# HarryShomer/LPFormer

Measured on AMD Instinct MI355X. Metric: candidate link-pairs scored/sec (whole node), higher is better.
Workload: dtype f32

## Files before the change

include/lpformer_hip.h:

```cpp
#ifndef LPFORMER_HIP_H
#define LPFORMER_HIP_H

#include <stdint.h>

#ifdef __cplusplus
extern "C" {
#endif

#define LPF_OK 0
#define LPF_ERR_INVALID (-1)
#define LPF_ERR_UNSUPPORTED (-2)
#define LPF_ERR_LAUNCH (-3)
#define LPF_ERR_NO_DEVICE (-4)

#define LPF_ABI_VERSION 16

#define LPF_FLAG_RELU 1u

int lpf_abi_version(void);
const char *lpf_strerror(int code);
const char *lpf_last_hip_error(void);
int lpf_device_info(int *cu_count, int *lds_bytes_per_cu, int *wave_size, char *arch_name, int arch_name_len);


// ... 89 lines not shown
                     const void *adj_cv, const void *a1_cv, const void *px_cv, const void *t0_cv, int32_t mode_cn,
                     int32_t use_px, void *desc, int64_t *offs, int32_t *item_pair, int64_t item_cap, int64_t *ctl,
                     uint64_t *plan_lb, void *stream);
int lpf_select3_run(int64_t bs, const void *desc, const int64_t *offs, const int32_t *item_pair, int64_t item_cap,
                    int64_t *ctl, uint64_t *run_lb, const void *u_cv, const void *mini, float th_cn, float th_1hop,
                    float th_non1hop, int32_t mode_cn, int32_t *type_ptr, void *entries, int64_t ent_cap,
                    int32_t grid_blocks, void *stream);

#define LPF_SELECT4_BLOCK 64
#define LPF_SELECT4_CTL_WORDS 32
int lpf_select4(int64_t bs, const int64_t *batch, int64_t batch_ld, int64_t n_nodes, const void *node_rec,
                const void *adj_cv, const void *a1_cv, const void *px_cv, const void *t0_cv, const void *u_cv,
                const void *mini, int32_t mode_cn, int32_t use_px, float th_cn, float th_1hop, float th_non1hop,
                int64_t *ctl, void *pair_tab, int32_t *blk_cnt, void *blk_types, void *entries, int64_t ent_cap,
                int32_t threads, void *stream);

int lpf_select4_regions(int64_t bs, const void *pair_tab, const void *blk_types, const void *entries4, int64_t ent_cap4,
                        int32_t *type_ptr, void *regions, int64_t ent_cap, int64_t *ctl, void *stream);

int lpf_select_export(int64_t bs, const int32_t *type_ptr, const void *entries, int64_t ent_cap, int64_t *type_ptr64,
                      float *counts_f, int64_t ldc, int32_t n_counts, int32_t *sel_pair, int32_t *sel_node,
                      float *sel_pa, float *sel_pb, void *stream);

int lpf_pair_scores_f32(int32_t D, const int64_t *type_ptr, int64_t bs, const int32_t *sel_pair,
                        const int32_t *sel_node, const float *sel_pa, const float *sel_pb,
                        const float *Z, int64_t ldz, const float *q, int64_t ldq,
                        const float *pe_tab, const float *pe_stat, const float *wfold_packed, const float *bfold,
                        const float *att, float *score, int64_t max_entries, void *stream);

int lpf_pair_softmax_gather_f32(int32_t D, int64_t bs, const int64_t *type_ptr, const int32_t *sel_node,
// ... 120 lines not shown
                                   float *pieces, int64_t units_cap, float *out, int64_t ldo, int32_t *perm,
                                   int64_t *n_nonempty, void *stream);

int lpf_tail_chain_rows_perm_f32(int64_t M, int32_t D, int32_t n_counts, const float *rows, int64_t ldrows,
                                 const float *wB_packed, const float *bB, const float *lnB_g, const float *lnB_b,
                                 const float *r_e, int64_t ldre, const float *wC_packed, const float *bC,
                                 const float *w_dot, const float *b_dot, const int64_t *sel_ctl, const int32_t *perm,
                                 const int64_t *n_full, const float *bC_empty, const float *row_empty, float *logit,
                                 float *prob, void *stream);
int lpf_tail_chain_rows_perm_bf16(int64_t M, int32_t D, int32_t n_counts, const float *rows, int64_t ldrows,
                                  const void *wB_packed_bf16, const float *bB, const float *lnB_g, const float *lnB_b,
                                  const float *r_e, int64_t ldre, const void *wC_packed_bf16, const float *bC,
                                  const float *w_dot, const float *b_dot, const int64_t *sel_ctl, const int32_t *perm,
                                  const int64_t *n_full, const float *bC_empty, const float *row_empty, float *logit,
                                  float *prob, void *stream);

int lpf_rowdot_sigmoid_f32(int64_t M, int32_t K, const float *A, int64_t lda, const float *w, float b,
                           float *logit, float *prob, void *stream);


int64_t lpf_ppr_push_workspace_bytes(int64_t n, int64_t n_waves, double alpha, double eps);

int lpf_ppr_push_f64(int64_t n, const int64_t *rowptr, const int32_t *col, double alpha, double eps,
                     int64_t n_waves, void *workspace, int64_t workspace_bytes, int32_t *pool_col, float *pool_val,
                     int64_t pool_capacity, int64_t *row_off, int32_t *row_len, int64_t *counters, void *stream);

int lpf_ppr_push_f64_sources(int64_t n, const int64_t *rowptr, const int32_t *col, int64_t n_src,
                             const int32_t *sources, double alpha, double eps, int64_t n_waves, void *workspace,
                             int64_t workspace_bytes, int32_t *pool_col, float *pool_val, int64_t pool_capacity,
                             int64_t *row_off, int32_t *row_len, int64_t *counters, void *stream);
// ... 149 lines not shown
```

lpformer_amd/csrc/select4.hip:

```cpp
#include "walk_common.h"

namespace {

using namespace walk;

constexpr int S4_PAIRS = LPF_SELECT4_BLOCK;
#ifndef S4_ROUNDS_N
#define S4_ROUNDS_N 4
#endif
constexpr int S4_ROUNDS = S4_ROUNDS_N;
constexpr int CTL_SLOTS = 1, CTL_ERR = 3, CTL_DONE = 10, CTL_ALLOC = 16;
constexpr int S4_SHARDS = 8;
static_assert(CTL_ALLOC + S4_SHARDS <= LPF_SELECT4_CTL_WORDS, "control block too small");

struct Args4 {
    int64_t bs;
    const int64_t *batch;
    int64_t batch_ld, n_nodes;
    const NodeRec *rec;
    const int2 *adj_cv, *a1_cv, *px_cv, *t0_cv;
    const int2 *u_cv;
    const uint32_t *mini;
    int32_t mode_cn, use_px;
    float th_cn, th_1, th_n;
    int64_t *ctl;
    int4 *pair_tab;
    int32_t *blk_cnt;
    int4 *blk_types;
    int4 *entries;
    int64_t ent_cap;
};

template <int NTH, int NB>
struct Lds4 {
    static constexpr int WAVES = NTH / 64, NR = WAVES * S4_ROUNDS, PAIRS = S4_PAIRS * NB;
    PairDesc3 dsc[PAIRS];
    uint4 flt[PAIRS][2][MINI_WORDS / 4];
    int32_t sflag[WAVES][S4_ROUNDS][64];
    int32_t loc[PAIRS];
    int32_t pcnt[PAIRS][4];
    int32_t rcnt[NR];
    int32_t sub[NB];
    int64_t base;
    int32_t run, ovf;
};
// ... 196 lines not shown
        for (int r = 0; r < S4_ROUNDS; ++r) {
            const int g = WAVES * r + wave;
            const int c3 = code[r] & 3;
            const int pos = L.rcnt[g < NR ? g : 0] + __popcll(keptb[r] & lt_mask);
            if (c3 && !ovf)
                A.entries[base + pos] = make_int4((int32_t)((uint32_t)(p0 + win[r]) | ((uint32_t)c3 << 29) |
                                                            ((code[r] & 4) ? FROM_B : 0u)),
                                                  node[r], __float_as_int(va[r]), __float_as_int(vb[r]));
            if (first[r]) L.pcnt[win[r]][3] = pos;
        }
    }
    S4_STAMP(8);
    lpf_lds_barrier();
    S4_STAMP(9);
    const bool ovf = S > 0 && L.ovf != 0;
    if (wave < NB) {
        const int j = S4_PAIRS * wave + lane;
        const int4 cc = *reinterpret_cast<const int4 *>(L.pcnt[j]);
        int kept = (j < np && !ovf) ? cc.x + cc.y + cc.z : 0;
        const int ne = __popcll(__ballot(kept > 0));
#pragma unroll
        for (int dlt = 32; dlt > 0; dlt >>= 1) kept += __shfl_xor(kept, dlt, 64);
        const int64_t blk = (int64_t)blockIdx.x * NB + wave;
        if (lane == 0 && blk * S4_PAIRS < A.bs) reinterpret_cast<int2 *>(A.blk_cnt)[blk] = make_int2(kept, ne);
        if (A.blk_types) {
            int c0 = (j < np && !ovf) ? cc.x : 0, c1 = (j < np && !ovf) ? cc.y : 0, c2 = (j < np && !ovf) ? cc.z : 0;
#pragma unroll
            for (int dlt = 32; dlt > 0; dlt >>= 1) {
                c0 += __shfl_xor(c0, dlt, 64);
                c1 += __shfl_xor(c1, dlt, 64);
                c2 += __shfl_xor(c2, dlt, 64);
            }
            if (lane == 0 && blk * S4_PAIRS < A.bs) A.blk_types[blk] = make_int4(c0, c1, c2, 0);
        }
    }
    if (tid < np) {
        const int4 c = *reinterpret_cast<const int4 *>(L.pcnt[tid]);
        A.pair_tab[p0 + tid] = ovf ? make_int4(0, 0, 0, 0) : make_int4((int32_t)(L.base + c.w), c.x, c.y, c.z);
    }
    if (tid == 0) {
        if (ovf) atomicOr(reinterpret_cast<unsigned long long *>(A.ctl + CTL_ERR), (unsigned long long)LPF_SELECT_ERR_ENTRY_CAP);
        const unsigned long long done = atomicAdd(reinterpret_cast<unsigned long long *>(A.ctl + CTL_DONE), 1ull);
        if (done == (unsigned long long)gridDim.x - 1ull) {
            unsigned long long most = 0ull, sum = 0ull;
            for (int sh = 0; sh < S4_SHARDS; ++sh) {
                const unsigned long long v = atomicExch(reinterpret_cast<unsigned long long *>(A.ctl + CTL_ALLOC + sh), 0ull);
                most = v > most ? v : most;
                sum += v;
            }
            atomicExch(reinterpret_cast<unsigned long long *>(A.ctl + CTL_DONE), 0ull);
            A.ctl[0] = (int64_t)(most * S4_SHARDS);
            A.ctl[CTL_SLOTS] = (int64_t)sum;
        }
// ... 4 lines not shown
        uint64_t *o = s4_stamp_buf + (int64_t)blockIdx.x * 16;
        for (int k = 0; k < 11; ++k) o[k] = st_t[k];
        o[11] = (uint64_t)S;
    }
#endif
}

}

#ifdef S4_STAMPS
extern "C" int lpf_select4_set_stamps(void *buf) {
    return hipMemcpyToSymbol(HIP_SYMBOL(s4_stamp_buf), &buf, sizeof(buf)) == hipSuccess ? LPF_OK : LPF_ERR_LAUNCH;
}
#endif

extern "C" int lpf_select4(int64_t bs, const int64_t *batch, int64_t batch_ld, int64_t n_nodes, const void *node_rec,
                           const void *adj_cv, const void *a1_cv, const void *px_cv, const void *t0_cv, const void *u_cv,
                           const void *mini, int32_t mode_cn, int32_t use_px, float th_cn, float th_1hop,
                           float th_non1hop, int64_t *ctl, void *pair_tab, int32_t *blk_cnt, void *blk_types,
                           void *entries, int64_t ent_cap, int32_t threads, void *stream) {
    if (bs == 0) return LPF_OK;
    LPF_REQUIRE(bs > 0 && bs < (1ll << 29) && batch && batch_ld >= bs && n_nodes > 0 && node_rec && adj_cv && a1_cv &&
                (px_cv || !use_px) && u_cv && mini && ctl && pair_tab && blk_cnt && entries && ent_cap > 0 &&
                ent_cap < (1ll << 31) && lpf_aligned16(node_rec) && lpf_aligned16(u_cv) && lpf_aligned16(mini) &&
                lpf_aligned16(pair_tab) && lpf_aligned16(entries) && (reinterpret_cast<uintptr_t>(blk_cnt) & 7) == 0 &&
                lpf_aligned16(blk_types));
    Args4 a;
    a.bs = bs; a.batch = batch; a.batch_ld = batch_ld; a.n_nodes = n_nodes;
    a.rec = static_cast<const NodeRec *>(node_rec);
    a.adj_cv = static_cast<const int2 *>(adj_cv); a.a1_cv = static_cast<const int2 *>(a1_cv);
    a.px_cv = static_cast<const int2 *>(px_cv); a.t0_cv = static_cast<const int2 *>(t0_cv);
    a.u_cv = static_cast<const int2 *>(u_cv); a.mini = static_cast<const uint32_t *>(mini);
    a.mode_cn = mode_cn; a.use_px = use_px; a.th_cn = th_cn; a.th_1 = th_1hop; a.th_n = th_non1hop;
    a.ctl = ctl; a.pair_tab = static_cast<int4 *>(pair_tab); a.blk_cnt = blk_cnt;
    a.blk_types = static_cast<int4 *>(blk_types);
    a.entries = static_cast<int4 *>(entries); a.ent_cap = ent_cap;
    const int64_t nb = (bs + S4_PAIRS - 1) / S4_PAIRS;
    hipStream_t s = static_cast<hipStream_t>(stream);
    if (threads == 0) {
        const int n_cu = lpf_cu_count();
        if (n_cu == 0) return LPF_ERR_NO_DEVICE;
        threads = 1024 + ((nb + 1) / 2 >= n_cu ? 4096 : 0);
    }
    const int nth = threads & 4095, per = threads / 4096 + 1;
    const dim3 grid((unsigned)((nb + per - 1) / per));
    if (nth == 1024 && per == 2) hipLaunchKernelGGL((select4_kernel<1024, 2>), grid, dim3(1024), 0, s, a);
    else if (nth == 1024 && per == 1) hipLaunchKernelGGL((select4_kernel<1024, 1>), grid, dim3(1024), 0, s, a);
    else if (nth == 1024 && per == 4) hipLaunchKernelGGL((select4_kernel<1024, 4>), grid, dim3(1024), 0, s, a);
    else if (nth == 512 && per == 1) hipLaunchKernelGGL((select4_kernel<512, 1>), grid, dim3(512), 0, s, a);
    else if (nth == 512 && per == 2) hipLaunchKernelGGL((select4_kernel<512, 2>), grid, dim3(512), 0, s, a);
    else if (nth == 256 && per == 1) hipLaunchKernelGGL((select4_kernel<256, 1>), grid, dim3(256), 0, s, a);
    else return LPF_ERR_INVALID;
    LPF_CHECK_LAUNCH();
    return LPF_OK;
}

namespace {

struct ArgsR {
    int64_t bs;
    const int4 *pair_tab, *blk_types, *entries4;
    int64_t ent_cap4;
    int32_t *type_ptr;
    int4 *regions;
    int64_t ent_cap;
    int64_t *ctl;
};

__global__ __launch_bounds__(64) void s4_regions_kernel(const ArgsR A) {
// ... 98 lines not shown
```

lpformer_amd/csrc/tail_chain.hip:

```cpp
#include <type_traits>

#include "lpf_common.h"

namespace {

typedef float f32x4 __attribute__((ext_vector_type(4)));

#ifndef LPF_TC_GROUPS
#define LPF_TC_GROUPS 4
#endif
constexpr int TC_GROUPS = LPF_TC_GROUPS;
constexpr int TC_WAVES = 2 * TC_GROUPS;
constexpr int TC_THREADS = 64 * TC_WAVES;

struct TailArgs {
    int64_t M;
    const float *x; int64_t ldx; int KA;
    const float *addend; int64_t ldadd;
    const float *wA, *lnA_g, *lnA_b; int NA;
    const float *tail; int64_t ldtail;
    const float *wB, *bB, *lnB_g, *lnB_b; int NB;
    const float *re; int64_t ldre;
    const float *wC, *bC; int NC;
    const float *wdot, *bdot;
    float *logit, *prob;
    const float *part;
    const float *bnd;
    int64_t units_cap;
    const int32_t *type_ptr;
    const float *att_bias;
    const int64_t *sel_ctl;
    int n_counts;
    const float *rows; int64_t ldrows;
    const int32_t *perm;
    const int64_t *n_full;
    const float *bC_empty;
    const float *row_empty;
};

constexpr int tc_per_thread(int ntp) { return (ntp * 64 + TC_THREADS - 1) / TC_THREADS; }
constexpr int tc_stage_stride(int ntp) { return (ntp * 64 + 511) / 512 * 512; }

typedef short bf16x4_bits __attribute__((ext_vector_type(4)));
template <int P, int NTP, typename T>
__device__ __forceinline__ void tc_load(T (&r)[P], const float *packed, int stage, int tid) {
    const T *src = reinterpret_cast<const T *>(packed) + (int64_t)stage * tc_stage_stride(NTP);
#pragma unroll
    for (int e = 0; e < P; ++e) {
        const int i = e * TC_THREADS + tid;
#ifdef TC_NOWLOAD
        r[e] = T{};
        (void)src; (void)i;
// ... 61 lines not shown
#pragma unroll
    for (int c = 0; c < TPW; ++c) {
        const f32x4 gg = *reinterpret_cast<const f32x4 *>(g + fbase + 16 * c);
        const f32x4 bb = *reinterpret_cast<const f32x4 *>(b + fbase + 16 * c);
        acc[c] = (acc[c] - mean) * rstd * gg + bb;
        if (relu) {
#pragma unroll
            for (int r = 0; r < 4; ++r) acc[c][r] = fmaxf(acc[c][r], 0.f);
        }
    }
}

#ifdef TC_STAMPS
__device__ uint64_t *tc_stamp_buf = nullptr;
#define TC_STAMP(k) do { if (lane == 0) st_t[k] = wall_clock64(); } while (0)
#define TC_STAMPS_OUT(kind) do { if (lane == 0 && tc_stamp_buf) { uint64_t *o__ = tc_stamp_buf + ((int64_t)blockIdx.x * TC_WAVES + wave) * 8; \
        for (int k__ = 0; k__ < 7; ++k__) o__[k__] = st_t[k__]; o__[7] = (kind); } } while (0)
#else
#define TC_STAMP(k) do { } while (0)
#define TC_STAMPS_OUT(kind) do { } while (0)
#endif

template <int NTA, int NTB, int NTC>
struct TcShape {
    static constexpr int NTPA = (NTA + 1) & ~1, NTPB = (NTB + 1) & ~1, NTPC = (NTC + 1) & ~1;
    static constexpr int PA = tc_per_thread(NTPA), PB = tc_per_thread(NTPB), PC = tc_per_thread(NTPC);
    static constexpr int PM = PA > PB ? (PA > PC ? PA : PC) : (PB > PC ? PB : PC);
    static constexpr int SLAB = PM * TC_THREADS;
    static constexpr int HT = NTPA > NTPB ? NTPA : NTPB;
    static constexpr int HID = TC_GROUPS * HT * 64;
    static constexpr size_t BYTES = (size_t)(2 * SLAB + HID) * sizeof(f32x4) + TC_WAVES * 16 * sizeof(float);
};

template <int NTA, int NTB, int NTC, int WM = 0, bool ROWS = false>
__global__ __launch_bounds__(TC_THREADS, NTC >= 32 ? 2 : (TC_THREADS >= 512 ? 4 : 3)) void tail_chain_kernel(const TailArgs A) {
    using S = TcShape<NTA, NTB, NTC>;
    constexpr bool WB = WM != 0;
    using WT = typename std::conditional<WM == 1, uint2, f32x4>::type;
    constexpr int NTPA = S::NTPA, NTPB = S::NTPB, NTPC = S::NTPC;
    constexpr int TPWA = NTPA / 2, TPWB = NTPB / 2, TPWC = NTPC / 2;
    constexpr int NGE = NTA;
    extern __shared__ __attribute__((aligned(16))) f32x4 lds[];
    f32x4 *hid = lds + 2 * S::SLAB;
    float *xch = reinterpret_cast<float *>(hid + S::HID);
    const int tid = threadIdx.x, lane = tid & 63, wave = tid >> 6;
    const int grp = wave >> 1, half = wave & 1, q = lane >> 4, j = lane & 15;
    float *my_x = xch + wave * 16 + j;
    const float *peer_x = xch + (wave ^ 1) * 16 + j;
    f32x4 *my_hid = hid + (grp * S::HT) * 64 + lane;
// ... 6 lines not shown
    const int64_t tile = blockIdx.x;
    const int64_t pos = tile * (16 * TC_GROUPS) + grp * 16 + j;
    const bool live = pos < A.M;
    bool lite = false;
    int64_t m = pos;
    if constexpr (ROWS) {
        if (A.perm) {
            m = A.perm[live ? pos : A.M - 1];
            lite = tile * (16 * TC_GROUPS) >= *A.n_full;
        }
    }
    const int64_t mm = live ? m : (ROWS && A.perm ? m : A.M - 1);
    bool no_sel = false;
    if constexpr (ROWS) no_sel = A.perm && A.row_empty && (live ? pos : A.M - 1) >= *A.n_full;

    if constexpr (ROWS) {
        if (lite) {
            f32x4 acc[TPWC];
#pragma unroll
            for (int c = 0; c < TPWC; ++c) acc[c] = (f32x4){0.f, 0.f, 0.f, 0.f};
            WT wr[S::PC];
            const float *rer = A.re + mm * A.ldre + 4 * q;
            tc_load<S::PC, NTPC>(wr, A.wC, 0, tid);
            f32x4 xr = *reinterpret_cast<const f32x4 *>(rer);
#pragma unroll 1
            for (int kg = 0; kg < NGE; ++kg) {
                const f32x4 bv = xr;
                WT *lw = reinterpret_cast<WT *>(lds) + buf * S::SLAB;
                tc_store<S::PC>(wr, lw, tid);
                __syncthreads();
                if (kg + 1 < NGE) {
                    tc_load<S::PC, NTPC>(wr, A.wC, kg + 1, tid);
                    xr = *reinterpret_cast<const f32x4 *>(rer + 16 * (kg + 1));
                }
                tc_mfma<TPWC>(acc, lw + (half * TPWC) * 64 + lane, bv);
                buf ^= 1;
            }
            const int fbase = 16 * half * TPWC + 4 * q;
            float d = 0.f;
#pragma unroll
            for (int c = 0; c < TPWC; ++c) {
                const f32x4 b = *reinterpret_cast<const f32x4 *>(A.bC_empty + fbase + 16 * c);
                const f32x4 w = *reinterpret_cast<const f32x4 *>(A.wdot + fbase + 16 * c);
#pragma unroll
                for (int r = 0; r < 4; ++r) d = fmaf(fmaxf(acc[c][r] + b[r], 0.f), w[r], d);
            }
            d = lpf_quad_sum(d);
            if (q == 0) *my_x = d;
            __syncthreads();
            if (live && q == 0 && half == 0) {
                d = d + *peer_x + A.bdot[0];
// ... 152 lines not shown
            }
        }
#pragma unroll
        for (int kg = 0; kg < NTPA + 1; ++kg) {
            WT *lw = reinterpret_cast<WT *>(lds) + buf * S::SLAB;
            tc_store<S::PB>(wrB, lw, tid);
            __syncthreads();
            if (kg + 1 < NTPA + 1) tc_load<S::PB, NTPB>(wrB, A.wB, kg + 1, tid);
            const f32x4 bv = kg < NTPA ? my_hid[(kg < NTPA ? kg : 0) * 64] : tailv;
            tc_mfma<TPWB>(accB, lw + (half * TPWB) * 64 + lane, bv, !((NTB & 1) && half == 1));
            buf ^= 1;
        }
    }
    TC_STAMP(2);
    WT wrC[S::PC];
    tc_load<S::PC, NTPC>(wrC, A.wC, 0, tid);
    const float *rer = A.re + mm * A.ldre + 4 * q;
    f32x4 xr = *reinterpret_cast<const f32x4 *>(rer);
    {
        const int fbase = 16 * half * TPWB + 4 * q;
#pragma unroll
        for (int c = 0; c < TPWB; ++c) accB[c] += *reinterpret_cast<const f32x4 *>(A.bB + fbase + 16 * c);
        tc_layernorm<TPWB>(accB, fbase, A.NB, A.lnB_g, A.lnB_b, half, q, my_x, peer_x, true);
#pragma unroll
        for (int c = 0; c < TPWB; ++c) my_hid[(half * TPWB + c) * 64] = accB[c];
    }

    TC_STAMP(3);
    f32x4 accC[TPWC];
#pragma unroll
    for (int c = 0; c < TPWC; ++c) accC[c] = (f32x4){0.f, 0.f, 0.f, 0.f};
#pragma unroll 1
    for (int kg = 0; kg < NGE; ++kg) {
        const f32x4 bv = xr;
        WT *lw = reinterpret_cast<WT *>(lds) + buf * S::SLAB;
        tc_store<S::PC>(wrC, lw, tid);
        __syncthreads();
        tc_load<S::PC, NTPC>(wrC, A.wC, kg + 1, tid);
        if (kg + 1 < NGE) xr = *reinterpret_cast<const f32x4 *>(rer + 16 * (kg + 1));
        tc_mfma<TPWC>(accC, lw + (half * TPWC) * 64 + lane, bv);
        buf ^= 1;
    }
    TC_STAMP(4);
#pragma unroll
    for (int kg = 0; kg < NTB; ++kg) {
        WT *lw = reinterpret_cast<WT *>(lds) + buf * S::SLAB;
        tc_store<S::PC>(wrC, lw, tid);
        __syncthreads();
        if (kg + 1 < NTB) tc_load<S::PC, NTPC>(wrC, A.wC, NGE + kg + 1, tid);
        tc_mfma<TPWC>(accC, lw + (half * TPWC) * 64 + lane, my_hid[kg * 64]);
        buf ^= 1;
    }
    TC_STAMP(5);
    {
        const int fbase = 16 * half * TPWC + 4 * q;
        float d = 0.f;
#pragma unroll
        for (int c = 0; c < TPWC; ++c) {
// ... 5 lines not shown
        d = lpf_quad_sum(d);
        __syncthreads();
        if (q == 0) *my_x = d;
        __syncthreads();
        if (live && q == 0 && half == 0) {
            d = d + *peer_x + A.bdot[0];
            if (A.sel_ctl && A.sel_ctl[3] != 0) d = __builtin_nanf("");
            if (A.logit) A.logit[m] = d;
            if (A.prob) A.prob[m] = 1.0f / (1.0f + expf(-d));
        }
    }
    TC_STAMP(6);
    TC_STAMPS_OUT(0);
}

template <int NTA, int NTB, int NTC, int WM = 0, bool ROWS = false>
int tc_launch(const TailArgs &a, hipStream_t s) {
    constexpr size_t lds = TcShape<NTA, NTB, NTC>::BYTES;
    auto kern = tail_chain_kernel<NTA, NTB, NTC, WM, ROWS>;
    LPF_SET_MAX_LDS(kern, lds);
    const int64_t blocks = (a.M + 16 * TC_GROUPS - 1) / (16 * TC_GROUPS);
    if (blocks > 0x7fffffff) return LPF_ERR_UNSUPPORTED;
    hipLaunchKernelGGL(kern, dim3((unsigned)blocks), dim3(TC_THREADS), lds, s, a);
    LPF_CHECK_LAUNCH();
    return LPF_OK;
}

}

#ifdef TC_STAMPS
extern "C" int lpf_tail_chain_set_stamps(void *buf) {
    return hipMemcpyToSymbol(HIP_SYMBOL(tc_stamp_buf), &buf, sizeof(buf)) == hipSuccess ? LPF_OK : LPF_ERR_LAUNCH;
}
#endif
// ... 137 lines not shown
    return tc_rows<0>(M, D, n_counts, rows, ldrows, wB_packed, bB, lnB_g, lnB_b, r_e, ldre, wC_packed, bC, w_dot, b_dot,
                          sel_ctl, logit, prob, stream, perm, n_full, bC_empty, row_empty);
}

extern "C" int lpf_tail_chain_rows_perm_bf16(int64_t M, int32_t D, int32_t n_counts, const float *rows, int64_t ldrows,
                                             const void *wB_packed_bf16, const float *bB, const float *lnB_g,
                                             const float *lnB_b, const float *r_e, int64_t ldre,
                                             const void *wC_packed_bf16, const float *bC, const float *w_dot,
                                             const float *b_dot, const int64_t *sel_ctl, const int32_t *perm,
                                             const int64_t *n_full, const float *bC_empty, const float *row_empty,
                                             float *logit, float *prob, void *stream) {
    LPF_REQUIRE(perm && n_full && bC_empty);
    return tc_rows<1>(M, D, n_counts, rows, ldrows, wB_packed_bf16, bB, lnB_g, lnB_b, r_e, ldre, wC_packed_bf16, bC, w_dot,
                         b_dot, sel_ctl, logit, prob, stream, perm, n_full, bC_empty, row_empty);
}
```

lpformer_amd/link_transformer.py:

```python
from __future__ import annotations

import functools
import math
import weakref
from typing import Optional

import numpy as np
import torch
import torch.nn as nn

from . import _lib, fold, graph, mask_delta, ops, patterns
from . import dist as lpf_dist
from ._lib import FLAG_RELU, check, ptr
from .ops import f32_rows, gemm, layernorm_, pad4, raw_stream
from .profile import KernelTimer


def _on_device(fn):
    @functools.wraps(fn)
    def wrapper(self, *args, **kwargs):
        idx = self.device.index if self.device.type == "cuda" else None
        if idx is None or not torch.cuda.is_available() or idx == torch.cuda.current_device():
            return fn(self, *args, **kwargs)
        with torch.cuda.device(idx):
# ... 485 lines not shown
        self.mask_delta_limit = 1 << 20
        self._delta_cache = None
        self.select_grid = 0
        self.select_blocks = True
        self.select4_threads = 0
        self.select4_regions = True
        self.use_side_stream = True
        self._side = None
        self.use_tail_chain = True
        self.use_fused_attention = True
        self.attention_impl = "auto"
        self.attention_rows = True
        self.flip_recheck_every = 16
        self._refolds = 0
        self.tail_skip_empty = True
        self.precision = "f32"
        self.encoder_precision = "f32"
        self.reuse_encoder_output = True
        self._enc_cache = None
        self.tail_precision = "f32"

    @property
    def _multi_head(self) -> bool:
        return int(self.train_args["num_heads"]) > 1 or self.num_layers > 1

    def _check_supported(self, train_ok: bool = False, heads_ok: bool = False):
        if self.num_layers > 2 or (self.num_layers == 2 and (int(self.train_args["num_heads"]) != 1 or self.dim > 128)):
            raise NotImplementedError("trans_layers = 1, or 2 with num_heads = 1 and dim <= 128: the reference's layer "
                                      "stack is shape-consistent for nothing else (link_transformer.py:55-62: the first "
                                      "of two layers is 2 dim wide, its halves feed the second)")
# ... 456 lines not shown
            return last[1]
        if self.training:
            return True
        ok = self._flip_stats()[1] <= self.PT_EXACT_MAX
        self._pt_choice = (self._folded[0], ok, self._refolds)
        return ok

    S4_SHAPE_SLOTS = (2000, 6000)

    def _select4_shape(self, bs: int, slots: int) -> int:
        nblk = (bs + _lib.SELECT4_BLOCK - 1) // _lib.SELECT4_BLOCK
        n_cu = torch.cuda.get_device_properties(self.device).multi_processor_count
        lo, hi = self.S4_SHAPE_SLOTS
        return 512 if (nblk >= 2 * n_cu and lo <= slots / max(nblk, 1) <= hi) else 0

    def _select4_launch(self, ws, batch, wi, regions: bool = False):
        lib, st = _lib.hip(), raw_stream(self.device)
        cn = 1 if self.mask == "cn" else 0
        with KernelTimer.span("select_run"):
            check(lib.lpf_select4(batch.shape[1], ptr(batch), batch.stride(0), self.num_nodes, ptr(wi.rec), ptr(wi.adj_cv),
                                  ptr(wi.a1_cv), ptr(wi.px_cv), ptr(wi.t0_cv), ptr(wi.u.cv), ptr(wi.mini), cn,
                                  1 if wi.use_px else 0, float(self.thresh_cn), float(self.thresh_1hop),
                                  float(self.thresh_non1hop), ptr(ws.ctl), ptr(ws.pair_tab), ptr(ws.blk_cnt),
                                  ptr(getattr(ws, "blk_types", None)), ptr(ws.entries4 if regions else ws.entries),
                                  ws.ent_cap4 if regions else ws.ent_cap,
                                  self.select4_threads or getattr(ws, "shape", 0), st), "lpf_select4")

    def _select4_device(self, batch: torch.Tensor, test_set: bool) -> "_Select4Workspace":
        st = raw_stream(self.device)
        bs = batch.shape[1]
        key = ("sel4", st, bs)
        ws = self._ws.get(key)
        if ws is None:
            ws = self._ws[key] = _Select4Workspace(self.device, bs)
        wi = self._select_graphs(test_set, None)
        if not ws.calibrated:
            ws.ensure(ent_cap=16)
            self._select4_launch(ws, batch, wi)
            err, need = ws.read_status()
            ws.shape = self._select4_shape(bs, int(ws.ctl[1].item()))
            ws.clear_errors()
            if err & _lib.SELECT_ERR_NODE_RANGE:
                raise IndexError(f"batch holds node ids outside [0, {self.num_nodes})")
            ws.ensure(ent_cap=3 * need[0] + 65536, shrink=True)
            self._select4_launch(ws, batch, wi)
            ws.kept_cap = 2 * ws.kept() + 65536
            ws.calibrated = True
        self._select4_launch(ws, batch, wi)
        return ws

    def check_selection(self, stream=None) -> bool:
        if stream is None:
            stream = torch.cuda.current_stream(self.device)
        st = stream.cuda_stream
        ok = True
        for key, ws in list(self._ws.items()):
            if not (isinstance(key, tuple) and key[0] in ("sel2", "sel4") and key[1] == st):
                continue
            err, _ = ws.read_status(stream)
            if err == 0:
                continue
            ok = False
            ws.clear_errors(stream)
# ... 313 lines not shown
            self._fold()
            last = getattr(self, "_auto_choice", None)
            if last is not None and (last[0] is self._folded[0] or self.training or
                                     self._refolds - last[2] < self.flip_recheck_every):
                return last[1]
            if self.training:
                return "flip"
            choice = "flip" if self.flips_per_entry() <= self.flip_break_even() else "mfma"
            self._auto_choice = (self._folded[0], choice, self._refolds)
            return choice
        return self.attention_impl

    def _uses_rows(self) -> bool:
        return self.attention_rows and self.attention_kernel() == "flip"

    def _attention_rows(self, batch, x_node, test_set, adj_mask, side, out, n_counts, order=False, q=None):
        lib, st, d = _lib.hip(), raw_stream(self.device), self.dim
        bs = batch.shape[1]
        w = self._fold()
        z = self._node_keys(x_node, w)
        if q is None:
            with torch.cuda.stream(side if side is not None else torch.cuda.current_stream(self.device)):
                q = self._pair_q(batch, x_node, w)
        four = self._uses_select4(adj_mask)
        ws = self._select4_device(batch, test_set) if four else self._select_device(batch, test_set, adj_mask)
        if side is not None:
            _lib.stream_wait(torch.cuda.current_stream(self.device), side)
        layer = self.att_layers[0]
        units_cap = (ws.kept_cap + 15) // 16 + 1 if four else (3 * ws.ent_cap + 15) // 16 + 1
        pieces = self._workspace("att_pieces", units_cap * 2 * int(lib.lpf_pair_rows_piece_floats(d)), torch.float32, st)
        extra = ()
        if order:
            perm = self._workspace("att_perm", bs, torch.int32, st)
            nfull = self._workspace("att_nfull", 1, torch.int64, st)
            extra = (ptr(perm), ptr(nfull)) if four else \
                (ptr(perm), ptr(self._zero_workspace("att_perm_lb", 2 * _lib.ROWS_PERM_LB_WORDS, st)), ptr(nfull))
        zt = self._z_bf16(z) if self.precision == "bf16" else z
        if four:
            pt = self._pattern_tables(w)
            geo = pt["geo"]
# ... 184 lines not shown
        self._check_supported(heads_ok=True)
        _require_gpu(X_node, "score_pairs")
        two_layer = (len(score_func.lins) == 2 and score_func.lins[1].out_features == 1 and
                     len(self.elementwise_lin.linears) == 2 and len(self.pairwise_lin.linears) == 2 and
                     not (score_func.training and score_func.dropout > 0))
        if not two_layer or self._multi_head:
            feats = self.pair_features(batch, X_node, test_set=test_set, adj_mask=adj_mask)
            return score_func.logits(feats) if logits else score_func(feats)
        self._fold_memo = None
        self._fold_memo = self._fold()
        try:
            return self._score_pairs_folded(batch, X_node, score_func, test_set, adj_mask, logits)
        finally:
            self._fold_memo = None

    def _score_pairs_folded(self, batch, X_node, score_func, test_set, adj_mask, logits):
        with torch.no_grad():
            d, pd = self.dim, self.dim + self.count_dim
            batch = self._prep_batch(batch)
            bs = batch.shape[1]
            x_node = f32_rows(X_node)
            a, c, kpad = self._score_fold(score_func)
            r = torch.empty(bs, kpad, dtype=torch.float32, device=self.device)
            ew, pw = self.elementwise_lin, self.pairwise_lin
            one_pass = d in (32, 64, 128, 256) and self.use_tail_chain and self.use_fused_attention and bs > 0
            q_side = None
            if one_pass and self.query_from == "table" and (d < 256 or self._uses_rows()):
                q_side = (self._node_y(x_node, self._fold()), torch.empty(bs, d, dtype=torch.float32, device=self.device))
            if one_pass:
                self._prepare_pair_major(adj_mask)
            side = self._fork()
            with torch.cuda.stream(side if side is not None else torch.cuda.current_stream(self.device)):
                t = ew._chain1.tables(ew.linears[0].weight, ew.linears[0].bias, ew.norm.weight, ew.norm.bias)
                if ew._chain1.run(t, x_node, relu=True, batch=batch, in_mode=1, out=r[:, :d], side=q_side) is None:
                    q_side = None
                    prod = torch.empty(bs, d, dtype=torch.float32, device=self.device)
                    ops.pair_gather(x_node, batch, product=prod, tag="pair_gather")
                    gemm(prod, ew._pads[0].get(ew.linears[0].weight), ew.linears[0].bias, out=r[:, :d], tag="gemm")
                    layernorm_(r[:, :d], ew.norm.weight, ew.norm.bias, relu=True, tag="layernorm")
            if (d in (32, 64, 128, 256) and self.use_tail_chain and self.use_fused_attention and bs > 0 and
# ... 134 lines not shown
```

Measured before the change: 251.1 million.

## Fuse query gather into select4 and elementwise stage into tail chain

```diff
diff --git a/include/lpformer_hip.h b/include/lpformer_hip.h
--- a/include/lpformer_hip.h
+++ b/include/lpformer_hip.h
@@ -127,6 +127,13 @@
                 const void *mini, int32_t mode_cn, int32_t use_px, float th_cn, float th_1hop, float th_non1hop,
                 int64_t *ctl, void *pair_tab, int32_t *blk_cnt, void *blk_types, void *entries, int64_t ent_cap,
                 int32_t threads, void *stream);
+
+int lpf_select4_q(int64_t bs, const int64_t *batch, int64_t batch_ld, int64_t n_nodes, const void *node_rec,
+                  const void *adj_cv, const void *a1_cv, const void *px_cv, const void *t0_cv, const void *u_cv,
+                  const void *mini, int32_t mode_cn, int32_t use_px, float th_cn, float th_1hop, float th_non1hop,
+                  int64_t *ctl, void *pair_tab, int32_t *blk_cnt, void *blk_types, void *entries, int64_t ent_cap,
+                  int32_t threads, const float *q_tab, int64_t ld_q_tab, float *q_out, int64_t ld_q_out, int32_t q_dim,
+                  void *stream);
 
 int lpf_select4_regions(int64_t bs, const void *pair_tab, const void *blk_types, const void *entries4, int64_t ent_cap4,
                         int32_t *type_ptr, void *regions, int64_t ent_cap, int64_t *ctl, void *stream);
@@ -277,6 +284,14 @@
                                   const float *w_dot, const float *b_dot, const int64_t *sel_ctl, const int32_t *perm,
                                   const int64_t *n_full, const float *bC_empty, const float *row_empty, float *logit,
                                   float *prob, void *stream);
+int lpf_tail_chain_rows_perm_ew_f32(int64_t M, int32_t D, int32_t n_counts, const float *rows, int64_t ldrows,
+                                    const float *wB_packed, const float *bB, const float *lnB_g, const float *lnB_b,
+                                    const float *r_e, int64_t ldre, const float *wC_packed, const float *bC,
+                                    const float *w_dot, const float *b_dot, const int64_t *sel_ctl, const int32_t *perm,
+                                    const int64_t *n_full, const float *bC_empty, const float *row_empty,
+                                    const float *X, int64_t ldx, const int64_t *batch, int64_t batch_ld, int64_t n_rows,
+                                    const float *wE_packed, const float *bE, const float *lnE_g, const float *lnE_b,
+                                    float *logit, float *prob, void *stream);
 
 int lpf_rowdot_sigmoid_f32(int64_t M, int32_t K, const float *A, int64_t lda, const float *w, float b,
                            float *logit, float *prob, void *stream);
diff --git a/lpformer_amd/csrc/select4.hip b/lpformer_amd/csrc/select4.hip
--- a/lpformer_amd/csrc/select4.hip
+++ b/lpformer_amd/csrc/select4.hip
@@ -29,6 +29,9 @@
     int4 *blk_types;
     int4 *entries;
     int64_t ent_cap;
+    const float *q_tab; int64_t ld_q_tab;
+    float *q_out; int64_t ld_q_out;
+    int32_t q_dim;
 };
 
 template <int NTH, int NB>
@@ -255,6 +258,45 @@
     lpf_lds_barrier();
     S4_STAMP(9);
     const bool ovf = S > 0 && L.ovf != 0;
+    constexpr int QU = 32 / WAVES, NU = NB * QU;
+    static_assert(32 % WAVES == 0, "a block's 32 units are dealt wavefront by wavefront");
+    const int hl = lane & 31, hh = lane >> 5;
+    const bool qcol = A.q_out && 4 * hl < A.q_dim;
+    int64_t qp[NU];
+    float4 qa[NU], qb[NU];
+#pragma unroll
+    for (int u = 0; u < NU; ++u) qp[u] = -1;
+    if (A.q_out) {
+#pragma unroll
+        for (int q = 0; q < NB; ++q) {
+            const int jq = S4_PAIRS * q + lane;
+            const int4 cq = *reinterpret_cast<const int4 *>(L.pcnt[jq]);
+            const bool ne = jq < np && !ovf && cq.x + cq.y + cq.z > 0;
+            const uint64_t bq = __ballot(ne);
+            const int nq = __popcll(bq), rank = __popcll(bq & lt_mask);
+#pragma unroll
+            for (int k = 0; k < QU; ++k) {
+                const int u = q * QU + k;
+                const int r0 = 2 * (wave + k * WAVES);
+                qa[u] = make_float4(0.f, 0.f, 0.f, 0.f); qb[u] = qa[u];
+                if (r0 < nq) {
+                    const uint64_t m0 = __ballot(ne && rank == r0), m1 = __ballot(ne && rank == r0 + 1);
+                    const uint64_t mine = hh ? m1 : m0;
+                    if (mine) {
+                        const int jm = S4_PAIRS * q + __builtin_ctzll(mine);
+                        const int64_t ia = L.dsc[jm].a, ib = L.dsc[jm].b;
+                        if ((uint64_t)ia < (uint64_t)A.n_nodes && (uint64_t)ib < (uint64_t)A.n_nodes) {
+                            qp[u] = p0 + jm;
+                            if (qcol) {
+                                qa[u] = *reinterpret_cast<const float4 *>(A.q_tab + ia * A.ld_q_tab + 4 * hl);
+                                qb[u] = *reinterpret_cast<const float4 *>(A.q_tab + ib * A.ld_q_tab + 4 * hl);
+                            }
+                        }
+                    }
+                }
+            }
+        }
+    }
     if (wave < NB) {
         const int j = S4_PAIRS * wave + lane;
         const int4 cc = *reinterpret_cast<const int4 *>(L.pcnt[j]);
@@ -278,6 +320,13 @@
     if (tid < np) {
         const int4 c = *reinterpret_cast<const int4 *>(L.pcnt[tid]);
         A.pair_tab[p0 + tid] = ovf ? make_int4(0, 0, 0, 0) : make_int4((int32_t)(L.base + c.w), c.x, c.y, c.z);
+    }
+    if (A.q_out) {
+#pragma unroll
+        for (int u = 0; u < NU; ++u)
+            if (qp[u] >= 0 && qcol)
+                *reinterpret_cast<float4 *>(A.q_out + qp[u] * A.ld_q_out + 4 * hl) =
+                    make_float4(qa[u].x + qb[u].x, qa[u].y + qb[u].y, qa[u].z + qb[u].z, qa[u].w + qb[u].w);
     }
     if (tid == 0) {
         if (ovf) atomicOr(reinterpret_cast<unsigned long long *>(A.ctl + CTL_ERR), (unsigned long long)LPF_SELECT_ERR_ENTRY_CAP);
@@ -312,17 +361,21 @@
 }
 #endif
 
-extern "C" int lpf_select4(int64_t bs, const int64_t *batch, int64_t batch_ld, int64_t n_nodes, const void *node_rec,
-                           const void *adj_cv, const void *a1_cv, const void *px_cv, const void *t0_cv, const void *u_cv,
-                           const void *mini, int32_t mode_cn, int32_t use_px, float th_cn, float th_1hop,
-                           float th_non1hop, int64_t *ctl, void *pair_tab, int32_t *blk_cnt, void *blk_types,
-                           void *entries, int64_t ent_cap, int32_t threads, void *stream) {
+extern "C" int lpf_select4_q(int64_t bs, const int64_t *batch, int64_t batch_ld, int64_t n_nodes, const void *node_rec,
+                             const void *adj_cv, const void *a1_cv, const void *px_cv, const void *t0_cv, const void *u_cv,
+                             const void *mini, int32_t mode_cn, int32_t use_px, float th_cn, float th_1hop,
+                             float th_non1hop, int64_t *ctl, void *pair_tab, int32_t *blk_cnt, void *blk_types,
+                             void *entries, int64_t ent_cap, int32_t threads, const float *q_tab, int64_t ld_q_tab,
+                             float *q_out, int64_t ld_q_out, int32_t q_dim, void *stream) {
     if (bs == 0) return LPF_OK;
     LPF_REQUIRE(bs > 0 && bs < (1ll << 29) && batch && batch_ld >= bs && n_nodes > 0 && node_rec && adj_cv && a1_cv &&
                 (px_cv || !use_px) && u_cv && mini && ctl && pair_tab && blk_cnt && entries && ent_cap > 0 &&
                 ent_cap < (1ll << 31) && lpf_aligned16(node_rec) && lpf_aligned16(u_cv) && lpf_aligned16(mini) &&
                 lpf_aligned16(pair_tab) && lpf_aligned16(entries) && (reinterpret_cast<uintptr_t>(blk_cnt) & 7) == 0 &&
                 lpf_aligned16(blk_types));
+    LPF_REQUIRE(!q_out || (q_tab && q_dim > 0 && (q_dim & 3) == 0 && ld_q_tab >= q_dim && ld_q_out >= q_dim &&
+                           (ld_q_tab & 3) == 0 && (ld_q_out & 3) == 0 && lpf_aligned16(q_tab) && lpf_aligned16(q_out)));
+    if (q_out && q_dim > 128) return LPF_ERR_UNSUPPORTED;
     Args4 a;
     a.bs = bs; a.batch = batch; a.batch_ld = batch_ld; a.n_nodes = n_nodes;
     a.rec = static_cast<const NodeRec *>(node_rec);
@@ -333,6 +386,7 @@
     a.ctl = ctl; a.pair_tab = static_cast<int4 *>(pair_tab); a.blk_cnt = blk_cnt;
     a.blk_types = static_cast<int4 *>(blk_types);
     a.entries = static_cast<int4 *>(entries); a.ent_cap = ent_cap;
+    a.q_tab = q_tab; a.ld_q_tab = ld_q_tab; a.q_out = q_out; a.ld_q_out = ld_q_out; a.q_dim = q_dim;
     const int64_t nb = (bs + S4_PAIRS - 1) / S4_PAIRS;
     hipStream_t s = static_cast<hipStream_t>(stream);
     if (threads == 0) {
@@ -351,6 +405,16 @@
     else return LPF_ERR_INVALID;
     LPF_CHECK_LAUNCH();
     return LPF_OK;
+}
+
+extern "C" int lpf_select4(int64_t bs, const int64_t *batch, int64_t batch_ld, int64_t n_nodes, const void *node_rec,
+                           const void *adj_cv, const void *a1_cv, const void *px_cv, const void *t0_cv, const void *u_cv,
+                           const void *mini, int32_t mode_cn, int32_t use_px, float th_cn, float th_1hop,
+                           float th_non1hop, int64_t *ctl, void *pair_tab, int32_t *blk_cnt, void *blk_types,
+                           void *entries, int64_t ent_cap, int32_t threads, void *stream) {
+    return lpf_select4_q(bs, batch, batch_ld, n_nodes, node_rec, adj_cv, a1_cv, px_cv, t0_cv, u_cv, mini, mode_cn, use_px,
+                         th_cn, th_1hop, th_non1hop, ctl, pair_tab, blk_cnt, blk_types, entries, ent_cap, threads, nullptr,
+                         0, nullptr, 0, 0, stream);
 }
 
 namespace {
diff --git a/lpformer_amd/csrc/tail_chain.hip b/lpformer_amd/csrc/tail_chain.hip
--- a/lpformer_amd/csrc/tail_chain.hip
+++ b/lpformer_amd/csrc/tail_chain.hip
@@ -36,6 +36,9 @@
     const int64_t *n_full;
     const float *bC_empty;
     const float *row_empty;
+    const float *X; int64_t ldX;
+    const int64_t *batch; int64_t batch_ld, n_rows;
+    const float *wE, *bE, *lnE_g, *lnE_b;
 };
 
 constexpr int tc_per_thread(int ntp) { return (ntp * 64 + TC_THREADS - 1) / TC_THREADS; }
@@ -127,8 +130,8 @@
 #ifdef TC_STAMPS
 __device__ uint64_t *tc_stamp_buf = nullptr;
 #define TC_STAMP(k) do { if (lane == 0) st_t[k] = wall_clock64(); } while (0)
-#define TC_STAMPS_OUT(kind) do { if (lane == 0 && tc_stamp_buf) { uint64_t *o__ = tc_stamp_buf + ((int64_t)blockIdx.x * TC_WAVES + wave) * 8; \
-        for (int k__ = 0; k__ < 7; ++k__) o__[k__] = st_t[k__]; o__[7] = (kind); } } while (0)
+#define TC_STAMPS_OUT(kind) do { if (lane == 0 && tc_stamp_buf) { uint64_t *o__ = tc_stamp_buf + ((int64_t)blockIdx.x * TC_WAVES + wave) * 16; \
+        for (int k__ = 0; k__ < 8; ++k__) o__[k__] = st_t[k__]; o__[15] = (kind); } } while (0)
 #else
 #define TC_STAMP(k) do { } while (0)
 #define TC_STAMPS_OUT(kind) do { } while (0)
@@ -145,7 +148,7 @@
     static constexpr size_t BYTES = (size_t)(2 * SLAB + HID) * sizeof(f32x4) + TC_WAVES * 16 * sizeof(float);
 };
 
-template <int NTA, int NTB, int NTC, int WM = 0, bool ROWS = false>
+template <int NTA, int NTB, int NTC, int WM = 0, bool ROWS = false, bool EW = false>
 __global__ __launch_bounds__(TC_THREADS, NTC >= 32 ? 2 : (TC_THREADS >= 512 ? 4 : 3)) void tail_chain_kernel(const TailArgs A) {
     using S = TcShape<NTA, NTB, NTC>;
     constexpr bool WB = WM != 0;
@@ -182,9 +185,66 @@
     bool no_sel = false;
     if constexpr (ROWS) no_sel = A.perm && A.row_empty && (live ? pos : A.M - 1) >= *A.n_full;
 
+    f32x4 accC[TPWC];
+    if constexpr (EW) {
+        static_assert(ROWS && WM == 0 && S::PA == 1 && NTPA == NTA && NGE % 2 == 0 && 2 * tc_stage_stride(NTPA) <= S::SLAB &&
+                          tc_stage_stride(2 * NTPA) == 2 * tc_stage_stride(NTPA), "stage E: the fp32 rows form at D = 128");
+        int64_t ra = A.batch[mm], rb = A.batch[A.batch_ld + mm];
+        if ((uint64_t)ra >= (uint64_t)A.n_rows) ra = 0;
+        if ((uint64_t)rb >= (uint64_t)A.n_rows) rb = 0;
+        const float *xa = A.X + ra * A.ldX + 4 * q, *xb = A.X + rb * A.ldX + 4 * q;
+        f32x4 accE[TPWA];
+#pragma unroll
+        for (int c = 0; c < TPWA; ++c) accE[c] = (f32x4){0.f, 0.f, 0.f, 0.f};
+        WT wrE[2];
+        tc_load<2, 2 * NTPA>(wrE, A.wE, 0, tid);
+        f32x4 xra[NGE], xrb[NGE];
+#pragma unroll
+        for (int kg = 0; kg < NGE; ++kg) {
+            xra[kg] = *reinterpret_cast<const f32x4 *>(xa + 16 * kg);
+            xrb[kg] = *reinterpret_cast<const f32x4 *>(xb + 16 * kg);
+        }
+#pragma unroll
+        for (int kg = 0; kg < NGE; kg += 2) {
+            const f32x4 bv0 = xra[kg] * xrb[kg], bv1 = xra[kg + 1] * xrb[kg + 1];
+            WT *lw = reinterpret_cast<WT *>(lds) + buf * S::SLAB;
+            tc_store<2>(wrE, lw, tid);
+            __syncthreads();
+            if (kg + 2 < NGE) tc_load<2, 2 * NTPA>(wrE, A.wE, kg / 2 + 1, tid);
+            tc_mfma<TPWA>(accE, lw + (half * TPWA) * 64 + lane, bv0);
+            tc_mfma<TPWA>(accE, lw + tc_stage_stride(NTPA) + (half * TPWA) * 64 + lane, bv1);
+            buf ^= 1;
+        }
+        WT wrCe[S::PC];
+        tc_load<S::PC, NTPC>(wrCe, A.wC, 0, tid);
+        {
+            const int fbase = 16 * half * TPWA + 4 * q;
+#pragma unroll
+            for (int c = 0; c < TPWA; ++c) accE[c] += *reinterpret_cast<const f32x4 *>(A.bE + fbase + 16 * c);
+            tc_layernorm<TPWA>(accE, fbase, A.NA, A.lnE_g, A.lnE_b, half, q, my_x, peer_x, true);
+#pragma unroll
+            for (int c = 0; c < TPWA; ++c) my_hid[(half * TPWA + c) * 64] = accE[c];
+        }
+        TC_STAMP(7);
+#pragma unroll
+        for (int c = 0; c < TPWC; ++c) accC[c] = (f32x4){0.f, 0.f, 0.f, 0.f};
+#pragma unroll 1
+        for (int kg = 0; kg < NGE; ++kg) {
+            WT *lw = reinterpret_cast<WT *>(lds) + buf * S::SLAB;
+            tc_store<S::PC>(wrCe, lw, tid);
+            __syncthreads();
+            if (kg + 1 < NGE) tc_load<S::PC, NTPC>(wrCe, A.wC, kg + 1, tid);
+            tc_mfma<TPWC>(accC, lw + (half * TPWC) * 64 + lane, my_hid[kg * 64]);
+            buf ^= 1;
+        }
+        TC_STAMP(4);
+        if (!lite) __syncthreads();
+    }
+
     if constexpr (ROWS) {
         if (lite) {
-            f32x4 acc[TPWC];
+            f32x4 (&acc)[TPWC] = accC;
+            if constexpr (!EW) {
 #pragma unroll
             for (int c = 0; c < TPWC; ++c) acc[c] = (f32x4){0.f, 0.f, 0.f, 0.f};
             WT wr[S::PC];
@@ -203,6 +263,7 @@
                 }
                 tc_mfma<TPWC>(acc, lw + (half * TPWC) * 64 + lane, bv);
                 buf ^= 1;
+            }
             }
             const int fbase = 16 * half * TPWC + 4 * q;
             float d = 0.f;
@@ -385,9 +446,10 @@
     }
     TC_STAMP(2);
     WT wrC[S::PC];
-    tc_load<S::PC, NTPC>(wrC, A.wC, 0, tid);
-    const float *rer = A.re + mm * A.ldre + 4 * q;
-    f32x4 xr = *reinterpret_cast<const f32x4 *>(rer);
+    tc_load<S::PC, NTPC>(wrC, A.wC, EW ? NGE : 0, tid);
+    const float *rer = EW ? nullptr : A.re + mm * A.ldre + 4 * q;
+    f32x4 xr = (f32x4){0.f, 0.f, 0.f, 0.f};
+    if constexpr (!EW) xr = *reinterpret_cast<const f32x4 *>(rer);
     {
         const int fbase = 16 * half * TPWB + 4 * q;
 #pragma unroll
@@ -398,7 +460,7 @@
     }
 
     TC_STAMP(3);
-    f32x4 accC[TPWC];
+    if constexpr (!EW) {
 #pragma unroll
     for (int c = 0; c < TPWC; ++c) accC[c] = (f32x4){0.f, 0.f, 0.f, 0.f};
 #pragma unroll 1
@@ -413,6 +475,7 @@
         buf ^= 1;
     }
     TC_STAMP(4);
+    }
 #pragma unroll
     for (int kg = 0; kg < NTB; ++kg) {
         WT *lw = reinterpret_cast<WT *>(lds) + buf * S::SLAB;
@@ -448,10 +511,10 @@
     TC_STAMPS_OUT(0);
 }
 
-template <int NTA, int NTB, int NTC, int WM = 0, bool ROWS = false>
+template <int NTA, int NTB, int NTC, int WM = 0, bool ROWS = false, bool EW = false>
 int tc_launch(const TailArgs &a, hipStream_t s) {
     constexpr size_t lds = TcShape<NTA, NTB, NTC>::BYTES;
-    auto kern = tail_chain_kernel<NTA, NTB, NTC, WM, ROWS>;
+    auto kern = tail_chain_kernel<NTA, NTB, NTC, WM, ROWS, EW>;
     LPF_SET_MAX_LDS(kern, lds);
     const int64_t blocks = (a.M + 16 * TC_GROUPS - 1) / (16 * TC_GROUPS);
     if (blocks > 0x7fffffff) return LPF_ERR_UNSUPPORTED;
@@ -619,3 +682,32 @@
     return tc_rows<1>(M, D, n_counts, rows, ldrows, wB_packed_bf16, bB, lnB_g, lnB_b, r_e, ldre, wC_packed_bf16, bC, w_dot,
                          b_dot, sel_ctl, logit, prob, stream, perm, n_full, bC_empty, row_empty);
 }
+
+extern "C" int lpf_tail_chain_rows_perm_ew_f32(int64_t M, int32_t D, int32_t n_counts, const float *rows, int64_t ldrows,
+                                               const float *wB_packed, const float *bB, const float *lnB_g,
+                                               const float *lnB_b, const float *r_e, int64_t ldre, const float *wC_packed,
+                                               const float *bC, const float *w_dot, const float *b_dot,
+                                               const int64_t *sel_ctl, const int32_t *perm, const int64_t *n_full,
+                                               const float *bC_empty, const float *row_empty, const float *X, int64_t ldx,
+                                               const int64_t *batch, int64_t batch_ld, int64_t n_rows,
+                                               const float *wE_packed, const float *bE, const float *lnE_g,
+                                               const float *lnE_b, float *logit, float *prob, void *stream) {
+    if (!wE_packed)
+        return lpf_tail_chain_rows_perm_f32(M, D, n_counts, rows, ldrows, wB_packed, bB, lnB_g, lnB_b, r_e, ldre, wC_packed, bC,
+                                            w_dot, b_dot, sel_ctl, perm, n_full, bC_empty, row_empty, logit, prob, stream);
+    if (M == 0) return LPF_OK;
+    if (D != 128) return LPF_ERR_UNSUPPORTED;
+    LPF_REQUIRE(perm && n_full && bC_empty && lpf_aligned16(bC_empty) && (!row_empty || lpf_aligned16(row_empty)));
+    LPF_REQUIRE(M > 0 && rows && wB_packed && bB && lnB_g && lnB_b && wC_packed && bC && w_dot && b_dot && (logit || prob));
+    LPF_REQUIRE((n_counts == 1 || n_counts == 3 || n_counts == 4) && (ldrows & 3) == 0 && ldrows >= D + 4);
+    LPF_REQUIRE(X && batch && bE && lnE_g && lnE_b && n_rows > 0 && batch_ld >= M && (ldx & 3) == 0 && ldx >= D);
+    LPF_REQUIRE(lpf_aligned16(rows) && lpf_aligned16(wB_packed) && lpf_aligned16(wC_packed) && lpf_aligned16(bB) &&
+                lpf_aligned16(lnB_g) && lpf_aligned16(lnB_b) && lpf_aligned16(bC) && lpf_aligned16(w_dot) &&
+                lpf_aligned16(X) && lpf_aligned16(wE_packed) && lpf_aligned16(bE) && lpf_aligned16(lnE_g) &&
+                lpf_aligned16(lnE_b));
+    TailArgs a{M, nullptr, 0, 0, nullptr, 0, nullptr, nullptr, nullptr, D, nullptr, 0, wB_packed, bB,
+               lnB_g, lnB_b, D + n_counts, nullptr, 0, wC_packed, bC, 2 * D, w_dot, b_dot, logit, prob,
+               nullptr, nullptr, 0, nullptr, nullptr, sel_ctl, n_counts, rows, ldrows, perm, n_full, bC_empty, row_empty,
+               X, ldx, batch, batch_ld, n_rows, wE_packed, bE, lnE_g, lnE_b};
+    return tc_launch<8, 9, 16, 0, true, true>(a, static_cast<hipStream_t>(stream));
+}
diff --git a/lpformer_amd/link_transformer.py b/lpformer_amd/link_transformer.py
--- a/lpformer_amd/link_transformer.py
+++ b/lpformer_amd/link_transformer.py
@@ -2,6 +2,7 @@
 
 import functools
 import math
+import os
 import weakref
 from typing import Optional
 
@@ -523,6 +524,7 @@
         self.flip_recheck_every = 16
         self._refolds = 0
         self.tail_skip_empty = True
+        self.fuse_step = False if os.environ.get("LPF_STEP_FORM") == "four" else "auto"
         self.precision = "f32"
         self.encoder_precision = "f32"
         self.reuse_encoder_output = True
@@ -1009,19 +1011,21 @@
         lo, hi = self.S4_SHAPE_SLOTS
         return 512 if (nblk >= 2 * n_cu and lo <= slots / max(nblk, 1) <= hi) else 0
 
-    def _select4_launch(self, ws, batch, wi, regions: bool = False):
+    def _select4_launch(self, ws, batch, wi, regions: bool = False, q=None):
         lib, st = _lib.hip(), raw_stream(self.device)
         cn = 1 if self.mask == "cn" else 0
+        name = "lpf_select4" if q is None else "lpf_select4_q"
+        extra = () if q is None else (ptr(q[0]), q[0].stride(0), ptr(q[1]), q[1].stride(0), q[1].shape[1])
         with KernelTimer.span("select_run"):
-            check(lib.lpf_select4(batch.shape[1], ptr(batch), batch.stride(0), self.num_nodes, ptr(wi.rec), ptr(wi.adj_cv),
-                                  ptr(wi.a1_cv), ptr(wi.px_cv), ptr(wi.t0_cv), ptr(wi.u.cv), ptr(wi.mini), cn,
-                                  1 if wi.use_px else 0, float(self.thresh_cn), float(self.thresh_1hop),
-                                  float(self.thresh_non1hop), ptr(ws.ctl), ptr(ws.pair_tab), ptr(ws.blk_cnt),
-                                  ptr(getattr(ws, "blk_types", None)), ptr(ws.entries4 if regions else ws.entries),
-                                  ws.ent_cap4 if regions else ws.ent_cap,
-                                  self.select4_threads or getattr(ws, "shape", 0), st), "lpf_select4")
-
-    def _select4_device(self, batch: torch.Tensor, test_set: bool) -> "_Select4Workspace":
+            check(getattr(lib, name)(batch.shape[1], ptr(batch), batch.stride(0), self.num_nodes, ptr(wi.rec), ptr(wi.adj_cv),
+                                     ptr(wi.a1_cv), ptr(wi.px_cv), ptr(wi.t0_cv), ptr(wi.u.cv), ptr(wi.mini), cn,
+                                     1 if wi.use_px else 0, float(self.thresh_cn), float(self.thresh_1hop),
+                                     float(self.thresh_non1hop), ptr(ws.ctl), ptr(ws.pair_tab), ptr(ws.blk_cnt),
+                                     ptr(getattr(ws, "blk_types", None)), ptr(ws.entries4 if regions else ws.entries),
+                                     ws.ent_cap4 if regions else ws.ent_cap,
+                                     self.select4_threads or getattr(ws, "shape", 0), *extra, st), name)
+
+    def _select4_device(self, batch: torch.Tensor, test_set: bool, q=None) -> "_Select4Workspace":
         st = raw_stream(self.device)
         bs = batch.shape[1]
         key = ("sel4", st, bs)
@@ -1041,7 +1045,7 @@
             self._select4_launch(ws, batch, wi)
             ws.kept_cap = 2 * ws.kept() + 65536
             ws.calibrated = True
-        self._select4_launch(ws, batch, wi)
+        self._select4_launch(ws, batch, wi, q=q)
         return ws
 
     def check_selection(self, stream=None) -> bool:
@@ -1385,16 +1389,21 @@
     def _uses_rows(self) -> bool:
         return self.attention_rows and self.attention_kernel() == "flip"
 
-    def _attention_rows(self, batch, x_node, test_set, adj_mask, side, out, n_counts, order=False, q=None):
+    def _attention_rows(self, batch, x_node, test_set, adj_mask, side, out, n_counts, order=False, q=None, q_tab=None):
         lib, st, d = _lib.hip(), raw_stream(self.device), self.dim
         bs = batch.shape[1]
         w = self._fold()
         z = self._node_keys(x_node, w)
+        four = self._uses_select4(adj_mask)
+        q_sel = None
+        if q_tab is not None:
+            assert four and q is None and side is None
+            q = self._workspace("att_q", bs * d, torch.float32, st)[:bs * d].view(bs, d)
+            q_sel = (q_tab, q)
         if q is None:
             with torch.cuda.stream(side if side is not None else torch.cuda.current_stream(self.device)):
                 q = self._pair_q(batch, x_node, w)
-        four = self._uses_select4(adj_mask)
-        ws = self._select4_device(batch, test_set) if four else self._select_device(batch, test_set, adj_mask)
+        ws = self._select4_device(batch, test_set, q=q_sel) if four else self._select_device(batch, test_set, adj_mask)
         if side is not None:
             _lib.stream_wait(torch.cuda.current_stream(self.device), side)
         layer = self.att_layers[0]
@@ -1609,6 +1618,40 @@
         finally:
             self._fold_memo = None
 
+    def _three_launches(self, x_node, adj_mask) -> bool:
+        ew = self.elementwise_lin
+        if self.fuse_step == "auto" and self.use_side_stream:
+            return False
+        return bool(self.fuse_step and self.dim == 128 and self.precision == "f32" and self.tail_precision == "f32" and
+                    self.query_from == "table" and self.tail_skip_empty and ew.norm is not None and
+                    tuple(ew.linears[0].weight.shape) == (128, 128) and x_node.shape[1] == 128 and
+                    x_node.stride(0) % 4 == 0 and x_node.data_ptr() % 16 == 0 and
+                    self._uses_rows() and self._uses_select4(adj_mask))
+
+    def _score_pairs_three(self, batch, x_node, score_func, test_set, a, c, logits):
+        lib, st, d = _lib.hip(), raw_stream(self.device), self.dim
+        bs = batch.shape[1]
+        ew = self.elementwise_lin
+        self._prepare_pair_major(None)
+        y = self._node_y(x_node, self._fold())
+        te = ew._chain1.tables(ew.linears[0].weight, ew.linears[0].bias, ew.norm.weight, ew.norm.bias)
+        rows = self._zero_workspace("att_rows", bs * (d + 4), st).view(bs, d + 4)
+        ws, perm, nfull = self._attention_rows(batch, x_node, test_set, None, None, rows, self.count_dim, order=True,
+                                               q_tab=y)
+        tt = self._tail_tables(score_func, a, c)
+        res = torch.empty(bs, dtype=torch.float32, device=self.device)
+        with KernelTimer.span("tail_chain"):
+            rc = lib.lpf_tail_chain_rows_perm_ew_f32(
+                bs, d, self.count_dim, ptr(rows), rows.stride(0), ptr(tt["wB"]), ptr(tt["bB"]), ptr(tt["lnB_g"]),
+                ptr(tt["lnB_b"]), None, 0, ptr(tt["wC"]), ptr(tt["bC"]), ptr(tt["w_dot"]), ptr(tt["b_dot"]), ptr(ws.ctl),
+                ptr(perm), ptr(nfull), ptr(tt["bC_empty"]), ptr(tt["row_empty"]), ptr(x_node), x_node.stride(0),
+                ptr(batch), batch.stride(0), x_node.shape[0], ptr(te["w1p"]), ptr(te["b1"]), ptr(te["ln_g"]),
+                ptr(te["ln_b"]), ptr(res) if logits else None, None if logits else ptr(res), st)
+        if rc == _lib.CONST["LPF_ERR_UNSUPPORTED"]:
+            return None
+        check(rc, "lpf_tail_chain_rows_perm_ew_f32")
+        return res
+
     def _score_pairs_folded(self, batch, X_node, score_func, test_set, adj_mask, logits):
         with torch.no_grad():
             d, pd = self.dim, self.dim + self.count_dim
@@ -1616,9 +1659,13 @@
             bs = batch.shape[1]
             x_node = f32_rows(X_node)
             a, c, kpad = self._score_fold(score_func)
-            r = torch.empty(bs, kpad, dtype=torch.float32, device=self.device)
             ew, pw = self.elementwise_lin, self.pairwise_lin
             one_pass = d in (32, 64, 128, 256) and self.use_tail_chain and self.use_fused_attention and bs > 0
+            if one_pass and self._three_launches(x_node, adj_mask):
+                res = self._score_pairs_three(batch, x_node, score_func, test_set, a, c, logits)
+                if res is not None:
+                    return res
+            r = torch.empty(bs, kpad, dtype=torch.float32, device=self.device)
             q_side = None
             if one_pass and self.query_from == "table" and (d < 256 or self._uses_rows()):
                 q_side = (self._node_y(x_node, self._fold()), torch.empty(bs, d, dtype=torch.float32, device=self.device))
```

Result: faster. 270.3 million (median of 6 runs) (+7.6%).
